# pyg-team/pyg-lib

Measured on AMD Instinct MI355X. Metric: segment_matmul GFLOP/s + sampled-edges/sec, 1/2/4/8 MI355X vs CPU ref, higher is better.
Workload: dtype bf16; 1 GPU; segment_matmul ogbn-mag-shaped: 154 relations, 21,111,007 rows, F_in=F_out=128 (BASELINE.json configs[1]); relations=154, rows=21111007, rows_per_gpu=21111007, F=128

## Files before the change

include/pyg_hip.h:

```cpp
#ifndef PYG_HIP_H_
#define PYG_HIP_H_

#include <stddef.h>
#include <stdint.h>

#ifdef __cplusplus
extern "C" {
#endif

#define PYG_HIP_API __attribute__((visibility("default")))

typedef enum {
  PYG_HIP_OK = 0,
  PYG_HIP_ERR_INVALID = -1,
  PYG_HIP_ERR_UNSUPPORTED = -2,
  PYG_HIP_ERR_RUNTIME = -3,
  PYG_HIP_ERR_WORKSPACE = -4
} pyg_hip_status;

typedef enum {
  PYG_F32 = 0,
  PYG_F64 = 1,
  PYG_F16 = 2,
  PYG_BF16 = 3,
  PYG_I8 = 4,
  PYG_U8 = 5,
  PYG_I16 = 6,
  PYG_I32 = 7,
  PYG_I64 = 8
} pyg_dtype;


#define PYG_HIP_ABI_VERSION 20
PYG_HIP_API int pyg_hip_abi_version(void);
PYG_HIP_API int64_t pyg_hip_version(void);
PYG_HIP_API const char* pyg_hip_last_error(void);
PYG_HIP_API const char* pyg_hip_arch(void);

PYG_HIP_API int pyg_hip_set_float_atomic_mode(int mode);
PYG_HIP_API const char* pyg_hip_last_accumulate_info(void);
PYG_HIP_API int pyg_hip_atomic_selftest(void* scratch, size_t scratch_bytes, int rounds, char* report, size_t report_cap,
                                        void* stream);


#define PYG_HIP_MM_SCHED_AUTO 0
#define PYG_HIP_MM_SCHED_CONTIGUOUS 1
#define PYG_HIP_MM_SCHED_CYCLIC 2
#define PYG_HIP_MM_SCHED_TICKET 3
#define PYG_HIP_MM_SCHED_GENERAL 4
#define PYG_HIP_MM_SCHED_NAIVE 5
#define PYG_HIP_MM_SCHED_RING 6
#define PYG_HIP_MM_SCHED_MASK 0xf
#define PYG_HIP_MM_F32_SPLIT 0x100

PYG_HIP_API size_t pyg_hip_matmul_workspace_size(int64_t num_groups);

// ... 45 lines not shown
} pyg_hip_rgcn_relation;

PYG_HIP_API size_t pyg_hip_rgcn_fused_workspace_size(int64_t num_relations, int64_t num_edges);

#define PYG_HIP_RGCN_CHECKED 1
#define PYG_HIP_RGCN_CAS 2
#define PYG_HIP_RGCN_DEFERRED 4
PYG_HIP_API int pyg_hip_rgcn_pending_error(void);
#define PYG_HIP_RGCN_GROUPED 8
PYG_HIP_API size_t pyg_hip_rgcn_grouped_workspace_size(const pyg_hip_rgcn_relation* relations, int64_t num_relations,
                                                       int64_t num_out_rows);
PYG_HIP_API int pyg_hip_rgcn_fused(int dtype, const void* x, int64_t num_x_rows, const pyg_hip_rgcn_relation* relations,
                                   int64_t num_relations, void* out, int64_t num_out_rows, int64_t K, int64_t M,
                                   int checked, void* workspace, size_t workspace_bytes, void* stream);
#define PYG_HIP_RGCN_ROUTE_UNSUPPORTED 0
#define PYG_HIP_RGCN_ROUTE_ATOMIC 1
#define PYG_HIP_RGCN_ROUTE_GROUPED_128 2
#define PYG_HIP_RGCN_ROUTE_GROUPED_SHAPE 3
#define PYG_HIP_RGCN_ROUTE_GROUPED_SMALL 4
#define PYG_HIP_RGCN_ROUTE_GROUPED_F32 5
#define PYG_HIP_RGCN_ROUTE_GROUPED_F32_SMALL 6
PYG_HIP_API int pyg_hip_rgcn_route(int dtype, int64_t K, int64_t M, int64_t num_relations, int flags);
PYG_HIP_API const char* pyg_hip_rgcn_last_route(void);


typedef struct {
  uint32_t state[624];
  int32_t left;
  uint32_t next;
} pyg_hip_mt19937;

typedef struct {
  void* user;
  void* (*alloc)(void* user, size_t bytes);
  void (*free)(void* user, void* ptr);
  void (*rng_blocks)(void* user, int64_t* words_host, int64_t num_blocks, int first);
  pyg_hip_mt19937* mt19937;
} pyg_hip_sampler_host;

typedef struct {
  const int64_t* rowptr;
  int64_t num_rows;
  const int64_t* col;
  int64_t num_cols;
  int32_t src_type;
  int32_t dst_type;
// ... 291 lines not shown
#define PYG_HIP_GRACLUS_TILE_SINGLE_THREADS 2
#define PYG_HIP_GRACLUS_TILE_SINGLE_MAX_NODES 3
#define PYG_HIP_GRACLUS_TILE_MULTI_THREADS 4
#define PYG_HIP_GRACLUS_TILE_BATCH 5
#define PYG_HIP_GRACLUS_TILE_SINGLE_MAX_EDGES 6
PYG_HIP_API int pyg_hip_graclus_route(int64_t N, int64_t E, int flags);
PYG_HIP_API const char* pyg_hip_graclus_last_route(void);
PYG_HIP_API int pyg_hip_graclus_tile(int which);
PYG_HIP_API size_t pyg_hip_graclus_workspace_size(int64_t N, int64_t E, int flags);
PYG_HIP_API int pyg_hip_graclus(const int64_t* rowptr, const int64_t* col, int weight_dtype, const void* weight, const int64_t* perm,
                                int64_t N, int64_t E, int flags, void* workspace, size_t workspace_bytes, int64_t* out, void* stream);
PYG_HIP_API int pyg_hip_graclus_pending_error(void);


PYG_HIP_API int pyg_hip_segment_csr(int op, int dtype, const void* src, const int64_t* indptr,
                                    int64_t indptr_slice_stride, void* out, int64_t* arg_out, int fresh,
                                    int64_t leading, int64_t rows, int64_t E, int64_t K, void* stream);

PYG_HIP_API size_t pyg_hip_csr_hub_workspace_size(int op, int dtype, int64_t leading, int64_t E, int64_t K);
PYG_HIP_API int pyg_hip_segment_csr_ws(int op, int dtype, const void* src, const int64_t* indptr,
                                       int64_t indptr_slice_stride, void* out, int64_t* arg_out, int fresh,
                                       int64_t leading, int64_t rows, int64_t E, int64_t K, void* workspace,
                                       size_t workspace_bytes, void* stream);

PYG_HIP_API int pyg_hip_gather_csr(int dtype, const void* src, const int64_t* indptr,
                                   int64_t indptr_slice_stride, void* out, int64_t leading, int64_t rows,
                                   int64_t E, int64_t K, void* stream);
PYG_HIP_API int pyg_hip_gather_csr_ws(int dtype, const void* src, const int64_t* indptr,
                                      int64_t indptr_slice_stride, void* out, int64_t leading, int64_t rows,
                                      int64_t E, int64_t K, void* workspace, size_t workspace_bytes, void* stream);

PYG_HIP_API int pyg_hip_softmax_csr(int dtype, const void* src, const int64_t* ptr, void* out, int64_t outer,
                                    int64_t D, int64_t inner, int64_t groups, void* stream);
PYG_HIP_API int pyg_hip_softmax_csr_backward(int dtype, const void* out, const void* out_grad,
                                             const int64_t* ptr, void* in_grad, int64_t outer, int64_t D,
                                             int64_t inner, int64_t groups, void* stream);

PYG_HIP_API const char* pyg_hip_csr_route(int family, int dtype, int64_t leading, int64_t rows, int64_t E, int64_t K,
                                          int flags, size_t workspace_bytes, unsigned misalign, int num_cus);
PYG_HIP_API const char* pyg_hip_csr_last_route(void);

PYG_HIP_API int64_t pyg_hip_hash_map_slots(int64_t n, double load_factor);
PYG_HIP_API int pyg_hip_hash_map_build(int key_dtype, const void* keys, int64_t n, uint64_t* table_keys,
                                       int64_t* table_vals, int64_t slots, int64_t* distinct_dev, void* stream);
PYG_HIP_API int pyg_hip_hash_map_get(int key_dtype, const void* query, int64_t m, const uint64_t* table_keys,
                                     const int64_t* table_vals, int64_t slots, int64_t* out, void* stream);
// ... 14 lines not shown
```

pyg_lib_amd/_capi.py:

```python
import ctypes
import os.path as osp

import torch

_HERE = osp.dirname(osp.abspath(__file__))
_LIB = None

OK = 0
ABI_VERSION = 20
DTYPES = {
    torch.float32: 0,
    torch.float64: 1,
    torch.float16: 2,
    torch.bfloat16: 3,
    torch.int8: 4,
    torch.uint8: 5,
    torch.int16: 6,
    torch.int32: 7,
    torch.int64: 8,
}


class Group(ctypes.Structure):
    _fields_ = [('input', ctypes.c_void_p), ('other', ctypes.c_void_p), ('out', ctypes.c_void_p),
                ('rows', ctypes.c_int64), ('k', ctypes.c_int32), ('m', ctypes.c_int32),
                ('other_trans', ctypes.c_int32), ('reserved', ctypes.c_int32)]


def lib_path() -> str:
    return osp.join(_HERE, 'libpyg_hip.so')


# ... 180 lines not shown
```

pyg_lib_amd/csrc/hip/csr.hip:

```cpp
#include "common.h"
#include "elem.h"
#include "csr_rows.h"

#include <algorithm>
#include <cstdint>
#include <type_traits>

namespace pyg_hip {
namespace {

enum { CSR_SUM = 0, CSR_MEAN = 1, CSR_MIN = 2, CSR_MAX = 3 };

template <typename T, int OP>
__device__ __forceinline__ typename Math<T>::acc_t minmax_identity() {
  return Math<T>::up(OP == CSR_MIN ? type_max<T>() : type_lowest<T>());
}

struct CsrShape {
  int64_t leading, rows, E, K;
  int64_t indptr_stride;
  int64_t long_cut = INT64_MAX;
  void* hub_ws = nullptr;
  size_t hub_ws_bytes = 0;
};
// ... 1176 lines not shown
}

size_t pyg_hip_csr_hub_workspace_size(int op, int dtype, int64_t leading, int64_t E, int64_t K) {
  CsrCall c{op, {}, leading, 0, E, K, false, 0, 0, 0, 0};
  if (leading < 0 || E < 0 || K <= 0 || op < 0 || op > CSR_GATHER || csr_type_of(dtype, &c.t) != PYG_HIP_OK) return 0;
  return csr_plan(c).ws_need;
}

int pyg_hip_segment_csr_ws(int op, int dtype, const void* src, const int64_t* indptr, int64_t indptr_slice_stride,
                           void* out, int64_t* arg_out, int fresh, int64_t leading, int64_t rows, int64_t E, int64_t K,
                           void* workspace, size_t workspace_bytes, void* stream_) {
  hipStream_t stream = static_cast<hipStream_t>(stream_);
  PYG_HIP_REQUIRE(leading >= 0 && rows >= 0 && E >= 0 && K >= 0, "segment_csr: negative size");
  if (csr_empty(CSR_SUM, leading, rows, E, K)) return note_empty();
  PYG_HIP_REQUIRE(op >= CSR_SUM && op <= CSR_MAX, "segment_csr: unknown reduction %d", op);
  PYG_HIP_REQUIRE(indptr && out && (src || E == 0), "segment_csr: NULL tensor");
  PYG_HIP_REQUIRE((op != CSR_MIN && op != CSR_MAX) || arg_out, "segment_csr: min/max need arg_out");
  PYG_HIP_REQUIRE(indptr_slice_stride == 0 || indptr_slice_stride >= rows + 1, "segment_csr: bad indptr stride");
  CsrShape s{leading, rows, E, K, indptr_slice_stride};
  s.hub_ws = workspace, s.hub_ws_bytes = workspace ? workspace_bytes : 0;
  PYG_DISPATCH_ALL(dtype, (run_segment<scalar_t>(op, src, indptr, nullptr, out, arg_out, fresh, s, stream)));
}

int pyg_hip_segment_csr(int op, int dtype, const void* src, const int64_t* indptr, int64_t indptr_slice_stride,
                        void* out, int64_t* arg_out, int fresh, int64_t leading, int64_t rows, int64_t E, int64_t K,
                        void* stream_) {
  return pyg_hip_segment_csr_ws(op, dtype, src, indptr, indptr_slice_stride, out, arg_out, fresh, leading, rows, E, K, nullptr, 0,
                                stream_);
}

int pyg_hip_gather_csr_ws(int dtype, const void* src, const int64_t* indptr, int64_t indptr_slice_stride, void* out,
                          int64_t leading, int64_t rows, int64_t E, int64_t K, void* workspace, size_t workspace_bytes,
                          void* stream_) {
  hipStream_t stream = static_cast<hipStream_t>(stream_);
  PYG_HIP_REQUIRE(leading >= 0 && rows >= 0 && E >= 0 && K >= 0, "gather_csr: negative size");
  if (csr_empty(CSR_GATHER, leading, rows, E, K)) return note_empty();
  PYG_HIP_REQUIRE(src && indptr && out, "gather_csr: NULL tensor");
  CsrShape s{leading, rows, E, K, indptr_slice_stride};
  s.hub_ws = workspace, s.hub_ws_bytes = workspace ? workspace_bytes : 0;
  PYG_DISPATCH_ALL(dtype, (run_gather_csr<scalar_t>(src, indptr, out, s, stream)));
}

int pyg_hip_gather_csr(int dtype, const void* src, const int64_t* indptr, int64_t indptr_slice_stride, void* out,
                       int64_t leading, int64_t rows, int64_t E, int64_t K, void* stream_) {
  return pyg_hip_gather_csr_ws(dtype, src, indptr, indptr_slice_stride, out, leading, rows, E, K, nullptr, 0, stream_);
}
// ... 25 lines not shown
```

pyg_lib_amd/rgcn.py:

```python
import os
import weakref
from typing import Dict, List, Optional, Tuple

import torch
from torch import Tensor
from torch.autograd.function import once_differentiable

from . import _capi, ops

EdgeType = Tuple[str, str, str]


def pending_index_error() -> int:
    return int(_capi.lib().pyg_hip_rgcn_pending_error())


_last_path = ['none']


def last_layer_path() -> str:
    return _last_path[0]


def last_layer_route() -> str:
# ... 66 lines not shown
    for et in edge_types:
        g, g_t, s, s_t = edge_roles(et, row_dict, col_dict, csc)
        counts.append(counts[-1] + g.numel())
        gather_idx.append(g + offsets[g_t] if offsets[g_t] else g)
        if num_out_rows is not None and s.numel() and not (x.is_cuda and torch.cuda.is_current_stream_capturing()):
            if int(s.max()) >= int(num_out_rows.get(s_t, 0)):
                raise RuntimeError(f"rgcn_layer: a scatter index of {et} is not below num_out_rows['{s_t}']")
        scatter_idx.append(s + ooff[s_t] if ooff[s_t] else s)
    total = ooff['__total__']
    if counts[-1] == 0:
        return x.new_zeros(total, weight.size(-1))
    gidx = torch.cat(gather_idx)
    sidx = torch.cat(scatter_idx)
    ptr = torch.tensor(counts, dtype=torch.long)
    feats = _GatherRows.apply(x, gidx)
    msgs = ops.segment_matmul(feats, ptr, weight)
    return ops.scatter_sum(msgs, sidx, dim=0, dim_size=total)


_DX_MODE = [os.environ.get('PYG_RGCN_DX', 'auto')]


def set_dx_mode(mode: str) -> str:
    if mode not in ('auto', 'grouped', 'atomic'):
        raise ValueError("dX mode must be 'auto', 'grouped' or 'atomic'")
    before, _DX_MODE[0] = _DX_MODE[0], mode
    return before


def _dx_grouped() -> bool:
    m = _DX_MODE[0]
    return m == 'grouped' or (m != 'atomic' and torch.are_deterministic_algorithms_enabled())


_ROUTE_ATOMIC, _FLAG_GROUPED = 1, 8


def _route(x: Tensor, weight: Tensor, relations: int, grouped: bool) -> int:
    code = _capi.DTYPES.get(x.dtype)
    if x.dim() != 2 or weight.dim() != 3 or code is None:
        return 0
    return _capi.lib().pyg_hip_rgcn_route(code, x.size(1), weight.size(2), relations, _FLAG_GROUPED if grouped else 0)


def _resolve_grouped(grouped: Optional[bool], scatter: List[Tensor]) -> bool:
    if grouped is None:
        from . import sampler
        grouped = all(sampler.rows_are_grouped(s) for s in scatter)
    return bool(grouped)


def _fusable(x: Tensor, weight: Tensor, grouped: bool = False, relations: int = 0) -> bool:
    if x.dim() != 2 or weight.dim() != 3:
        return False
    return (x.is_cuda and weight.size(1) == x.size(1) and weight.dtype == x.dtype and weight.device == x.device and
# ... 25 lines not shown


_transposed: Dict[Tuple, Tuple] = {}


def _transposed_sample(gather: List[Tensor], scatter: List[Tensor], gather_rows: int):
    key = tuple((id(t), t._version) for t in gather) + tuple((id(t), t._version) for t in scatter)
    hit = _transposed.get(key)
    if hit is not None and all(r() is t for r, t in zip(hit[0], list(gather) + list(scatter))):
        return hit[1], hit[2]
    counts = [g.numel() for g in gather]
    R = len(gather)
    keys = torch.cat([g + r * gather_rows if r else g for r, g in enumerate(gather)])
    skeys, perm = ops.index_sort(keys, max_value=max(R * gather_rows, 1))
    g_sorted = list(torch.split(skeys % gather_rows if R > 1 else skeys, counts))
    s_perm = list(torch.split(torch.cat(scatter)[perm], counts))
    if len(_transposed) >= 8:
        _transposed.pop(next(iter(_transposed)))
    refs = [weakref.ref(t) for t in list(gather) + list(scatter)]
    _transposed[key] = (refs, g_sorted, s_perm)
    return g_sorted, s_perm


def _dx_scatter(grad_out: Tensor, weight: Tensor, gather: List[Tensor], scatter: List[Tensor], goff: List[int],
                soff: List[int], rows: int, grows: Optional[List[int]] = None) -> Tensor:
    wt = weight.transpose(1, 2).contiguous()
    E = sum(g.numel() for g in gather)
    if E == 0:
        return grad_out.new_zeros(rows, weight.size(1))
    if _dx_grouped() and _fusable(grad_out, wt, True, len(gather)):
        g_sorted, s_perm = _transposed_sample(gather, scatter, rows)
        gx = grad_out.new_empty(rows, weight.size(1))
        torch.ops.pyg.rgcn_fused(grad_out, s_perm, g_sorted, soff, goff, wt, gx, True, grows)
        return gx
    if torch.are_deterministic_algorithms_enabled() or _route(grad_out, wt, len(gather), False) != _ROUTE_ATOMIC:
        ptr, gidx, sidx = _rel_ptr_and_indices(gather, scatter, goff, soff)
        msgs = ops.segment_matmul(ops.gather_coo(grad_out, sidx), ptr, wt)
        return ops.scatter_sum(msgs, gidx, dim=0, dim_size=rows)
    gx = grad_out.new_zeros(rows, weight.size(1))
    torch.ops.pyg.rgcn_fused(grad_out, scatter, gather, soff, goff, wt, gx)
    return gx


class _RGCNFused(torch.autograd.Function):

    @staticmethod
    def forward(ctx, x, weight, total, goff, soff, grouped, srows, grows, *index):
        R = len(index) // 2
        gather, scatter = list(index[:R]), list(index[R:])
        out = _fresh_out(x, total, weight.size(-1), grouped)
        torch.ops.pyg.rgcn_fused(x, gather, scatter, goff, soff, weight, out, grouped, srows)
        ctx.save_for_backward(x, weight, *index)
        ctx.meta = (goff, soff, R, grows)
        return out

    @staticmethod
    @once_differentiable
    def backward(ctx, grad_out):
        x, weight = ctx.saved_tensors[:2]
        index = ctx.saved_tensors[2:]
        goff, soff, R, grows = ctx.meta
        gather, scatter = list(index[:R]), list(index[R:])
        grad_out = grad_out.contiguous()
        gx = gw = None
        if ctx.needs_input_grad[0]:
            gx = _dx_scatter(grad_out, weight, gather, scatter, goff, soff, x.size(0), grows)
        if ctx.needs_input_grad[1]:
            ptr, gidx, sidx = _rel_ptr_and_indices(gather, scatter, goff, soff)
            if gidx.numel() == 0:
                gw = torch.zeros_like(weight)
            else:
                gw = torch.ops.pyg.segment_matmul_grad_other(ops.gather_coo(x, gidx), ptr, ops.gather_coo(grad_out, sidx))
        return (gx, gw, None, None, None, None, None, None) + (None,) * len(index)


class _RGCNFusedTables(torch.autograd.Function):

    @staticmethod
    def forward(ctx, weight, T, gtype, soff, grouped, out_rows, srows, *tensors):
        feat, node_id = list(tensors[:T]), list(tensors[T:2 * T])
        index = tensors[2 * T:]
        R = len(index) // 2
        gather, scatter = list(index[:R]), list(index[R:])
        n_t = [t.numel() for t in node_id]
        out = _fresh_out(feat[0], out_rows, weight.size(-1), grouped)
        torch.ops.pyg.rgcn_fused_tables(feat, node_id, gtype, gather, scatter, soff, weight, out, grouped, srows)
        ctx.save_for_backward(weight, *tensors)
        ctx.meta = (T, gtype, soff, R, n_t)
        return out

    @staticmethod
    @once_differentiable
    def backward(ctx, grad_out):
        weight = ctx.saved_tensors[0]
        tensors = ctx.saved_tensors[1:]
        T, gtype, soff, R, n_t = ctx.meta
        feat, node_id = list(tensors[:T]), list(tensors[T:2 * T])
        index = tensors[2 * T:]
        gather, scatter = list(index[:R]), list(index[R:])
        grad_out = grad_out.contiguous()
        toff = [0]
        for n in n_t:
            toff.append(toff[-1] + n)
        goff = [toff[t] for t in gtype]
        gw = None
        gfeat = [None] * T
        if ctx.needs_input_grad[0]:
            ptr, gidx, sidx = _rel_ptr_and_indices(gather, scatter, goff, soff)
            if gidx.numel() == 0:
                gw = torch.zeros_like(weight)
            else:
                xb = torch.cat([f[n] for f, n in zip(feat, node_id)])
                gw = torch.ops.pyg.segment_matmul_grad_other(ops.gather_coo(xb, gidx), ptr, ops.gather_coo(grad_out, sidx))
        if any(ctx.needs_input_grad[7 + t] for t in range(T)):
            gx = _dx_scatter(grad_out, weight, gather, scatter, goff, soff, toff[-1], [max(n_t[t], 1) for t in gtype])
            for t in range(T):
                if ctx.needs_input_grad[7 + t]:
                    gfeat[t] = torch.zeros_like(feat[t]).index_add_(0, node_id[t], gx[toff[t]:toff[t + 1]])
        return (gw, None, None, None, None, None, None) + tuple(gfeat) + (None,) * (len(tensors) - T)


def rgcn_layer_fused(x: Tensor, offsets: Dict[str, int], row_dict: Dict[EdgeType, Tensor],
                     col_dict: Dict[EdgeType, Tensor], edge_types: List[EdgeType], weight: Tensor,
                     csc: bool = False, grouped: Optional[bool] = None,
                     num_out_rows: Optional[Dict[str, int]] = None) -> Tensor:
    ooff = out_offsets(offsets, num_out_rows)
    total = ooff['__total__']
    roles = [edge_roles(et, row_dict, col_dict, csc) for et in edge_types]
    grouped = _resolve_grouped(grouped, [r[2] for r in roles]) and _fusable(x, weight, True, len(roles))
    if not (grouped or _fusable(x, weight, False, len(roles))) or (torch.are_deterministic_algorithms_enabled() and not grouped):
        return rgcn_layer(x, offsets, row_dict, col_dict, edge_types, weight, csc, num_out_rows)
    gather, scatter = [r[0] for r in roles], [r[2] for r in roles]
    goff, soff = [offsets[r[1]] for r in roles], [ooff[r[3]] for r in roles]
    srows = _scatter_rows(ooff, roles, edge_types)
    _last_path[0] = 'grouped' if grouped else 'atomic'
    if torch.is_grad_enabled() and (x.requires_grad or weight.requires_grad):
        trows = _type_rows(offsets)
        grows = [max(trows[r[1]], 1) for r in roles]
# ... 34 lines not shown
```

Baseline: 397,200 GFLOP/s.

## Compute RGCN backward dW and dX over scatter-row runs instead of per-edge

Adds a run-decomposition kernel that groups consecutive edges sharing a scatter row (capped at 32 per run). dW pre-sums gathered x rows per run and multiplies by one grad_out row per run, and dX multiplies grad_out once per run and then does a CSR index-sum over source rows. The intent is to cut per-edge GEMM rows and gathers in the backward pass, at the cost of new indexing kernels and cached run metadata keyed on tensor identity. It only touches the RGCN fused backward, not the segment_matmul forward throughput being measured.

```diff
diff --git a/include/pyg_hip.h b/include/pyg_hip.h
--- a/include/pyg_hip.h
+++ b/include/pyg_hip.h
@@ -31,7 +31,7 @@
 } pyg_dtype;
 
 
-#define PYG_HIP_ABI_VERSION 20
+#define PYG_HIP_ABI_VERSION 21
 PYG_HIP_API int pyg_hip_abi_version(void);
 PYG_HIP_API int64_t pyg_hip_version(void);
 PYG_HIP_API const char* pyg_hip_last_error(void);
@@ -123,6 +123,14 @@
 #define PYG_HIP_RGCN_ROUTE_GROUPED_F32_SMALL 6
 PYG_HIP_API int pyg_hip_rgcn_route(int dtype, int64_t K, int64_t M, int64_t num_relations, int flags);
 PYG_HIP_API const char* pyg_hip_rgcn_last_route(void);
+
+PYG_HIP_API size_t pyg_hip_rgcn_runs_workspace_size(int64_t num_edges);
+PYG_HIP_API int pyg_hip_rgcn_runs(const pyg_hip_rgcn_relation* relations, int64_t num_relations, int64_t max_len,
+                                  int64_t* run_ptr, int64_t* run_row, int64_t* rel_run_ptr, int32_t* run_of_edge,
+                                  int64_t* gather_rows, void* workspace, size_t workspace_bytes, void* stream);
+PYG_HIP_API int pyg_hip_rgcn_run_rows(int dtype, const void* x, int64_t num_x_rows, int64_t K, const int64_t* gather_rows,
+                                      const int64_t* run_ptr, const int64_t* run_row, int64_t num_runs, const void* grad_out,
+                                      int64_t num_out_rows, int64_t M, float* agg, float* grow, void* stream);
 
 
 typedef struct {
@@ -460,6 +468,9 @@
                                        int64_t indptr_slice_stride, void* out, int64_t* arg_out, int fresh,
                                        int64_t leading, int64_t rows, int64_t E, int64_t K, void* workspace,
                                        size_t workspace_bytes, void* stream);
+PYG_HIP_API int pyg_hip_segment_csr_index_sum(int dtype, const void* src, const int64_t* index, const int64_t* indptr, void* out,
+                                              int64_t rows, int64_t E, int64_t K, void* workspace, size_t workspace_bytes,
+                                              void* stream);
 
 PYG_HIP_API int pyg_hip_gather_csr(int dtype, const void* src, const int64_t* indptr,
                                    int64_t indptr_slice_stride, void* out, int64_t leading, int64_t rows,
diff --git a/pyg_lib_amd/_capi.py b/pyg_lib_amd/_capi.py
--- a/pyg_lib_amd/_capi.py
+++ b/pyg_lib_amd/_capi.py
@@ -7,7 +7,7 @@
 _LIB = None
 
 OK = 0
-ABI_VERSION = 20
+ABI_VERSION = 21
 DTYPES = {
     torch.float32: 0,
     torch.float64: 1,
diff --git a/pyg_lib_amd/csrc/binding/pyg_binding_rgcn_runs.cpp b/pyg_lib_amd/csrc/binding/pyg_binding_rgcn_runs.cpp
--- /dev/null
+++ b/pyg_lib_amd/csrc/binding/pyg_binding_rgcn_runs.cpp
@@ -0,0 +1,223 @@
+#include <ATen/ATen.h>
+#include <torch/library.h>
+
+#include <tuple>
+#include <vector>
+
+#include "binding_common.h"
+
+namespace pyg_amd {
+namespace {
+
+using Runs = std::tuple<Tensor, Tensor, Tensor, Tensor, Tensor>;
+
+int64_t check_runs(const at::TensorList scatter_index, at::IntArrayRef scatter_offset, const at::TensorList gather_index,
+                   at::IntArrayRef gather_offset, int64_t max_len) {
+  const size_t R = scatter_index.size();
+  TORCH_CHECK(R > 0 && gather_index.size() == R && scatter_offset.size() == R && gather_offset.size() == R,
+              "rgcn_runs: one scatter / gather index vector and offset per relation expected (at least one relation)");
+  TORCH_CHECK(max_len >= 1, "rgcn_runs: max_len must be positive");
+  int64_t E = 0;
+  for (size_t r = 0; r < R; ++r) {
+    for (const Tensor* t : {&scatter_index[r], &gather_index[r]})
+      TORCH_CHECK(t->dim() == 1 && t->scalar_type() == at::kLong && t->device() == scatter_index[0].device(),
+                  "rgcn_runs: index vectors must be 1-D int64 tensors on one device");
+    TORCH_CHECK(scatter_index[r].numel() == gather_index[r].numel(), "rgcn_runs: index vectors of a relation differ in length");
+    E += scatter_index[r].numel();
+  }
+  return E;
+}
+
+void check_dw_runs(const Tensor& x, const Tensor& gather_rows, const Tensor& grad_out, const Tensor& run_ptr, const Tensor& run_row,
+                   const Tensor& rel_run_ptr, int64_t num_runs) {
+  TORCH_CHECK(x.dim() == 2 && grad_out.dim() == 2 && x.scalar_type() == grad_out.scalar_type() && x.device() == grad_out.device(),
+              "rgcn_dw_runs: expected x [N, K] and grad_out [N_out, M] of one type on one device");
+  TORCH_CHECK(x.scalar_type() == at::kBFloat16 || x.scalar_type() == at::kHalf || x.scalar_type() == at::kFloat,
+              "rgcn_dw_runs: float32 / bfloat16 / float16 only (got ", x.scalar_type(), ")");
+  for (const Tensor* t : {&gather_rows, &run_ptr, &run_row, &rel_run_ptr})
+    TORCH_CHECK(t->dim() == 1 && t->scalar_type() == at::kLong && t->device() == x.device() && t->is_contiguous(),
+                "rgcn_dw_runs: gather_rows, run_ptr, run_row and rel_run_ptr must be contiguous int64 vectors on the device of x");
+  TORCH_CHECK(num_runs >= 0 && num_runs <= gather_rows.numel() && run_ptr.numel() > num_runs && run_row.numel() >= num_runs &&
+                  rel_run_ptr.numel() >= 1,
+              "rgcn_dw_runs: expected gather_rows [E >= P], run_ptr [> P], run_row [>= P], rel_run_ptr [R + 1]");
+  TORCH_CHECK(x.size(0) > 0 && grad_out.size(0) > 0 || num_runs == 0, "rgcn_dw_runs: runs over tensors without rows");
+}
+
+void check_dx_runs(const Tensor& grad_out, const Tensor& weight, const Tensor& run_row, const Tensor& rel_run_ptr, int64_t num_runs,
+                   const Tensor& src_index, const Tensor& indptr, int64_t rows) {
+  TORCH_CHECK(grad_out.dim() == 2 && weight.dim() == 3 && weight.size(2) == grad_out.size(1) &&
+                  weight.scalar_type() == grad_out.scalar_type() && weight.device() == grad_out.device(),
+              "rgcn_dx_runs: expected grad_out [N_out, M] and weight [R, K, M] of one type on one device");
+  TORCH_CHECK(grad_out.scalar_type() == at::kBFloat16 || grad_out.scalar_type() == at::kHalf || grad_out.scalar_type() == at::kFloat,
+              "rgcn_dx_runs: float32 / bfloat16 / float16 only (got ", grad_out.scalar_type(), ")");
+  for (const Tensor* t : {&run_row, &rel_run_ptr, &src_index, &indptr})
+    TORCH_CHECK(t->dim() == 1 && t->scalar_type() == at::kLong && t->device() == grad_out.device() && t->is_contiguous(),
+                "rgcn_dx_runs: run_row, rel_run_ptr, src_index and indptr must be contiguous int64 vectors on the device of grad_out");
+  TORCH_CHECK(num_runs >= 0 && run_row.numel() >= num_runs && rel_run_ptr.numel() == weight.size(0) + 1 && rows >= 0 &&
+                  indptr.numel() == rows + 1 && (num_runs == 0 || grad_out.size(0) > 0),
+              "rgcn_dx_runs: expected run_row [>= P], rel_run_ptr [R + 1], indptr [rows + 1]");
+}
+
+Runs rgcn_runs_kernel(const at::TensorList scatter_index, at::IntArrayRef scatter_offset, const at::TensorList gather_index,
+                      at::IntArrayRef gather_offset, int64_t max_len) {
+  PYG_TRACE("pyg::rgcn_runs");
+  const int64_t E = check_runs(scatter_index, scatter_offset, gather_index, gather_offset, max_len);
+  const size_t R = scatter_index.size();
+  const Tensor& like = scatter_index[0];
+  DeviceGuard guard(like.device());
+  std::vector<pyg_hip_rgcn_relation> rels(R);
+  std::vector<Tensor> keep;
+  for (size_t r = 0; r < R; ++r) {
+    keep.push_back(scatter_index[r].contiguous());
+    keep.push_back(gather_index[r].contiguous());
+    rels[r] = pyg_hip_rgcn_relation{};
+    rels[r].scatter_index = keep[2 * r].data_ptr<int64_t>();
+    rels[r].gather_index = keep[2 * r + 1].data_ptr<int64_t>();
+    rels[r].num_edges = keep[2 * r].numel();
+    rels[r].scatter_offset = scatter_offset[r];
+    rels[r].gather_offset = gather_offset[r];
+  }
+  const auto longs = like.options().dtype(at::kLong);
+  Tensor run_ptr = at::empty({E + 1}, longs), run_row = at::empty({E}, longs), rel_run_ptr = at::empty({(int64_t)R + 1}, longs);
+  Tensor run_of_edge = at::empty({E}, longs.dtype(at::kInt)), gather_rows = at::empty({E}, longs);
+  Tensor ws = at::empty({(int64_t)pyg_hip_rgcn_runs_workspace_size(E)}, longs.dtype(at::kByte));
+  check_status(pyg_hip_rgcn_runs(rels.data(), (int64_t)R, max_len, run_ptr.data_ptr<int64_t>(), run_row.data_ptr<int64_t>(),
+                                 rel_run_ptr.data_ptr<int64_t>(), run_of_edge.data_ptr<int32_t>(), gather_rows.data_ptr<int64_t>(),
+                                 ws.data_ptr(), (size_t)ws.numel(), current_stream(like)));
+  return {run_ptr, run_row, rel_run_ptr, run_of_edge, gather_rows};
+}
+
+Tensor rgcn_dw_runs_kernel(const Tensor& x, const Tensor& gather_rows, const Tensor& grad_out, const Tensor& run_ptr,
+                           const Tensor& run_row, const Tensor& rel_run_ptr, int64_t num_runs) {
+  PYG_TRACE("pyg::rgcn_dw_runs");
+  check_dw_runs(x, gather_rows, grad_out, run_ptr, run_row, rel_run_ptr, num_runs);
+  const int64_t R = rel_run_ptr.numel() - 1, K = x.size(1), M = grad_out.size(1), P = num_runs;
+  if (R == 0 || P == 0) return at::zeros({R, K, M}, x.options());
+  DeviceGuard guard(x.device());
+  const Tensor xc = x.contiguous(), gc = grad_out.contiguous();
+  const auto floats = x.options().dtype(at::kFloat);
+  Tensor agg = at::empty({P, K}, floats), grow = at::empty({P, M}, floats), dw = at::empty({R, K, M}, floats);
+  check_status(pyg_hip_rgcn_run_rows(dtype_code(x.scalar_type()), xc.data_ptr(), xc.size(0), K, gather_rows.data_ptr<int64_t>(),
+                                     run_ptr.data_ptr<int64_t>(), run_row.data_ptr<int64_t>(), P, gc.data_ptr(), gc.size(0), M,
+                                     agg.data_ptr<float>(), grow.data_ptr<float>(), current_stream(x)));
+  Tensor ws = at::empty({(int64_t)pyg_hip_segment_matmul_dw_workspace_size(R, K, M)}, floats.dtype(at::kByte));
+  check_status(pyg_hip_segment_matmul_dw(PYG_F32, agg.data_ptr(), rel_run_ptr.data_ptr<int64_t>(), 1, grow.data_ptr(), dw.data_ptr(),
+                                         P, K, M, R, ws.data_ptr(), (size_t)ws.numel(), current_stream(x)));
+  return dw.to(x.scalar_type());
+}
+
+Tensor rgcn_dx_runs_kernel(const Tensor& grad_out, const Tensor& weight, const Tensor& run_row, const Tensor& rel_run_ptr,
+                           int64_t num_runs, const Tensor& src_index, const Tensor& indptr, int64_t rows) {
+  PYG_TRACE("pyg::rgcn_dx_runs");
+  check_dx_runs(grad_out, weight, run_row, rel_run_ptr, num_runs, src_index, indptr, rows);
+  const int64_t R = weight.size(0), K = weight.size(1), M = weight.size(2), P = num_runs, E = src_index.numel();
+  if (rows == 0 || K == 0 || P == 0 || E == 0) return at::zeros({rows, K}, grad_out.options());
+  DeviceGuard guard(grad_out.device());
+  const int dt = dtype_code(grad_out.scalar_type());
+  const Tensor gc = grad_out.contiguous(), wt = weight.transpose(1, 2).contiguous();
+  Tensor gst = at::empty({P, M}, gc.options()), T = at::empty({P, K}, gc.options()), dx = at::empty({rows, K}, gc.options());
+  check_status(pyg_hip_gather_coo(dt, gc.data_ptr(), run_row.data_ptr<int64_t>(), gst.data_ptr(), 1, P, M, gc.size(0), current_stream(gc)));
+  const auto bytes = gc.options().dtype(at::kByte);
+  Tensor ws = at::empty({(int64_t)pyg_hip_matmul_workspace_size(R)}, bytes);
+  check_status(pyg_hip_segment_matmul(dt, gst.data_ptr(), rel_run_ptr.data_ptr<int64_t>(), 1, wt.data_ptr(), nullptr, T.data_ptr(), P, M, K, R,
+                                      ws.data_ptr(), (size_t)ws.numel(), 0, current_stream(gc)));
+  Tensor hub = at::empty({(int64_t)pyg_hip_csr_hub_workspace_size(0, dt, 1, E, K)}, bytes);
+  check_status(pyg_hip_segment_csr_index_sum(dt, T.data_ptr(), src_index.data_ptr<int64_t>(), indptr.data_ptr<int64_t>(), dx.data_ptr(),
+                                             rows, E, K, hub.numel() ? hub.data_ptr() : nullptr, (size_t)hub.numel(), current_stream(gc)));
+  return dx;
+}
+
+Tensor rgcn_dx_runs_cpu(const Tensor& grad_out, const Tensor& weight, const Tensor& run_row, const Tensor& rel_run_ptr,
+                        int64_t num_runs, const Tensor& src_index, const Tensor& indptr, int64_t rows) {
+  check_dx_runs(grad_out, weight, run_row, rel_run_ptr, num_runs, src_index, indptr, rows);
+  const int64_t R = weight.size(0), K = weight.size(1), P = num_runs;
+  if (rows == 0 || K == 0 || P == 0 || src_index.numel() == 0) return at::zeros({rows, K}, grad_out.options());
+  const Tensor gst = grad_out.index_select(0, run_row.narrow(0, 0, P)).to(at::kFloat);
+  const int64_t* rel = rel_run_ptr.data_ptr<int64_t>();
+  std::vector<Tensor> parts;
+  for (int64_t r = 0; r < R; ++r)
+    parts.push_back(at::matmul(gst.narrow(0, rel[r], rel[r + 1] - rel[r]), weight[r].to(at::kFloat).t()));
+  const Tensor T = at::cat(parts).to(grad_out.scalar_type()).to(at::kFloat);
+  const Tensor row_of = at::repeat_interleave(at::arange(rows, indptr.options()), indptr.narrow(0, 1, rows) - indptr.narrow(0, 0, rows));
+  return at::zeros({rows, K}, gst.options()).index_add_(0, row_of, T.index_select(0, src_index)).to(grad_out.scalar_type());
+}
+
+Runs rgcn_runs_cpu(const at::TensorList scatter_index, at::IntArrayRef scatter_offset, const at::TensorList gather_index,
+                   at::IntArrayRef gather_offset, int64_t max_len) {
+  const int64_t E = check_runs(scatter_index, scatter_offset, gather_index, gather_offset, max_len);
+  const size_t R = scatter_index.size();
+  const auto longs = scatter_index[0].options().dtype(at::kLong);
+  Tensor run_ptr = at::zeros({E + 1}, longs), run_row = at::zeros({E}, longs), rel_run_ptr = at::zeros({(int64_t)R + 1}, longs);
+  Tensor run_of_edge = at::zeros({E}, longs.dtype(at::kInt)), gather_rows = at::zeros({E}, longs);
+  int64_t* rp = run_ptr.data_ptr<int64_t>();
+  int64_t* rr = run_row.data_ptr<int64_t>();
+  int64_t* rel = rel_run_ptr.data_ptr<int64_t>();
+  int32_t* roe = run_of_edge.data_ptr<int32_t>();
+  int64_t* gr = gather_rows.data_ptr<int64_t>();
+  int64_t P = 0, pos = 0;
+  for (size_t r = 0; r < R; ++r) {
+    const Tensor s = scatter_index[r].contiguous(), g = gather_index[r].contiguous();
+    const int64_t* sp = s.data_ptr<int64_t>();
+    const int64_t* gp = g.data_ptr<int64_t>();
+    rel[r] = P;
+    int64_t first = 0;
+    for (int64_t j = 0; j < s.numel(); ++j, ++pos) {
+      if (j == 0 || sp[j] != sp[j - 1]) first = j;
+      if ((j - first) % max_len == 0) {
+        rp[P] = pos;
+        rr[P] = sp[j] + scatter_offset[r];
+        ++P;
+      }
+      roe[pos] = (int32_t)(P - 1);
+      gr[pos] = gp[j] + gather_offset[r];
+    }
+  }
+  rel[R] = P;
+  rp[P] = E;
+  return {run_ptr, run_row, rel_run_ptr, run_of_edge, gather_rows};
+}
+
+Tensor rgcn_dw_runs_cpu(const Tensor& x, const Tensor& gather_rows, const Tensor& grad_out, const Tensor& run_ptr,
+                        const Tensor& run_row, const Tensor& rel_run_ptr, int64_t num_runs) {
+  check_dw_runs(x, gather_rows, grad_out, run_ptr, run_row, rel_run_ptr, num_runs);
+  const int64_t R = rel_run_ptr.numel() - 1, K = x.size(1), M = grad_out.size(1), P = num_runs;
+  if (R == 0 || P == 0) return at::zeros({R, K, M}, x.options());
+  const Tensor ptr = run_ptr.narrow(0, 0, P + 1);
+  const Tensor run_id = at::repeat_interleave(at::arange(P, ptr.options()), ptr.narrow(0, 1, P) - ptr.narrow(0, 0, P));
+  const Tensor rows = x.to(at::kFloat).index_select(0, gather_rows.narrow(0, 0, run_id.numel()));
+  const Tensor agg = at::zeros({P, K}, x.options().dtype(at::kFloat)).index_add_(0, run_id, rows);
+  const Tensor grow = grad_out.to(at::kFloat).index_select(0, run_row.narrow(0, 0, P));
+  const int64_t* rel = rel_run_ptr.data_ptr<int64_t>();
+  std::vector<Tensor> parts;
+  for (int64_t r = 0; r < R; ++r)
+    parts.push_back(at::matmul(agg.narrow(0, rel[r], rel[r + 1] - rel[r]).t(), grow.narrow(0, rel[r], rel[r + 1] - rel[r])));
+  return at::stack(parts).to(x.scalar_type());
+}
+
+}
+
+TORCH_LIBRARY_FRAGMENT(pyg, m) {
+  m.def(TORCH_SELECTIVE_SCHEMA(
+      "pyg::rgcn_runs(Tensor[] scatter_index, int[] scatter_offset, Tensor[] gather_index, int[] gather_offset, int max_len) -> "
+      "(Tensor, Tensor, Tensor, Tensor, Tensor)"));
+  m.def(TORCH_SELECTIVE_SCHEMA(
+      "pyg::rgcn_dw_runs(Tensor x, Tensor gather_rows, Tensor grad_out, Tensor run_ptr, Tensor run_row, Tensor rel_run_ptr, "
+      "int num_runs) -> Tensor"));
+  m.def(TORCH_SELECTIVE_SCHEMA(
+      "pyg::rgcn_dx_runs(Tensor grad_out, Tensor weight, Tensor run_row, Tensor rel_run_ptr, int num_runs, Tensor src_index, "
+      "Tensor indptr, int rows) -> Tensor"));
+}
+
+TORCH_LIBRARY_IMPL(pyg, CUDA, m) {
+  m.impl(TORCH_SELECTIVE_NAME("pyg::rgcn_runs"), TORCH_FN(rgcn_runs_kernel));
+  m.impl(TORCH_SELECTIVE_NAME("pyg::rgcn_dw_runs"), TORCH_FN(rgcn_dw_runs_kernel));
+  m.impl(TORCH_SELECTIVE_NAME("pyg::rgcn_dx_runs"), TORCH_FN(rgcn_dx_runs_kernel));
+}
+
+TORCH_LIBRARY_IMPL(pyg, CPU, m) {
+  m.impl(TORCH_SELECTIVE_NAME("pyg::rgcn_runs"), TORCH_FN(rgcn_runs_cpu));
+  m.impl(TORCH_SELECTIVE_NAME("pyg::rgcn_dw_runs"), TORCH_FN(rgcn_dw_runs_cpu));
+  m.impl(TORCH_SELECTIVE_NAME("pyg::rgcn_dx_runs"), TORCH_FN(rgcn_dx_runs_cpu));
+}
+
+}
diff --git a/pyg_lib_amd/csrc/hip/csr.hip b/pyg_lib_amd/csrc/hip/csr.hip
--- a/pyg_lib_amd/csrc/hip/csr.hip
+++ b/pyg_lib_amd/csrc/hip/csr.hip
@@ -1222,6 +1222,15 @@
   PYG_DISPATCH_ALL(dtype, (run_segment<scalar_t>(op, src, indptr, nullptr, out, arg_out, fresh, s, stream)));
 }
 
+int pyg_hip_segment_csr_index_sum(int dtype, const void* src, const int64_t* index, const int64_t* indptr, void* out,
+                                  int64_t rows, int64_t E, int64_t K, void* workspace, size_t workspace_bytes, void* stream_) {
+  hipStream_t stream = static_cast<hipStream_t>(stream_);
+  PYG_HIP_REQUIRE(rows >= 0 && E >= 0 && K >= 0, "segment_csr_index_sum: negative size");
+  if (csr_empty(CSR_SUM, 1, rows, E, K)) return note_empty();
+  PYG_HIP_REQUIRE(indptr && out && ((src && index) || E == 0), "segment_csr_index_sum: NULL tensor");
+  return segment_csr_sum(dtype, src, indptr, 0, index, out, 1, rows, E, K, 1, stream, workspace, workspace ? workspace_bytes : 0);
+}
+
 int pyg_hip_segment_csr(int op, int dtype, const void* src, const int64_t* indptr, int64_t indptr_slice_stride,
                         void* out, int64_t* arg_out, int fresh, int64_t leading, int64_t rows, int64_t E, int64_t K,
                         void* stream_) {
diff --git a/pyg_lib_amd/csrc/hip/rgcn_runs.hip b/pyg_lib_amd/csrc/hip/rgcn_runs.hip
--- /dev/null
+++ b/pyg_lib_amd/csrc/hip/rgcn_runs.hip
@@ -0,0 +1,253 @@
+#include "csr_rows.h"
+#include "scan.h"
+
+namespace pyg_hip {
+namespace {
+
+constexpr int kRunsMaxRel = 32;
+constexpr int kRunsRowBits = 40;
+constexpr int64_t kRunsRowMask = (1LL << kRunsRowBits) - 1;
+
+struct RunsRel {
+  const int64_t* scatter[kRunsMaxRel];
+  const int64_t* gather[kRunsMaxRel];
+  int64_t soff[kRunsMaxRel], goff[kRunsMaxRel];
+  int64_t start[kRunsMaxRel + 1];
+};
+
+__global__ __launch_bounds__(256) void runs_keys_kernel(RunsRel t, int64_t E, int64_t* __restrict__ keys,
+                                                        int64_t* __restrict__ gather_rows) {
+  const int64_t i = (int64_t)blockIdx.x * 256 + threadIdx.x;
+  if (i >= E) return;
+  const int64_t* s = t.scatter[0];
+  const int64_t* g = t.gather[0];
+  int64_t so = t.soff[0], go = t.goff[0], st = t.start[0], rel = 0;
+#pragma unroll
+  for (int r = 1; r < kRunsMaxRel; ++r) {
+    const bool in = i >= t.start[r];
+    s = in ? t.scatter[r] : s;
+    g = in ? t.gather[r] : g;
+    so = in ? t.soff[r] : so;
+    go = in ? t.goff[r] : go;
+    st = in ? t.start[r] : st;
+    rel = in ? r : rel;
+  }
+  keys[i] = (rel << kRunsRowBits) | ((s[i - st] + so) & kRunsRowMask);
+  if (gather_rows) gather_rows[i] = g[i - st] + go;
+}
+
+struct MaxOp {
+  __host__ __device__ int64_t operator()(int64_t a, int64_t b) const { return a > b ? a : b; }
+  __host__ __device__ static int64_t identity() { return -1; }
+};
+
+struct StretchLoad {
+  const int64_t* keys;
+  __device__ int64_t operator()(int64_t i) const { return (i == 0 || keys[i] != keys[i - 1]) ? i : -1; }
+};
+struct StretchStore {
+  int64_t* first;
+  __device__ void operator()(int64_t i, int64_t before, int64_t v) const { first[i] = v > before ? v : before; }
+};
+
+struct RunLoad {
+  const int64_t* first;
+  int64_t max_len;
+  __device__ int64_t operator()(int64_t i) const { return (i - first[i]) % max_len == 0 ? 1 : 0; }
+};
+struct RunStore {
+  const int64_t* keys;
+  int64_t* run_ptr;
+  int64_t* run_row;
+  int64_t* rel_run_ptr;
+  int32_t* run_of_edge;
+  __device__ void operator()(int64_t i, int64_t before, int64_t v) const {
+    run_of_edge[i] = (int32_t)(before + v - 1);
+    if (v == 0) return;
+    const int64_t key = keys[i];
+    run_ptr[before] = i;
+    run_row[before] = key & kRunsRowMask;
+    const int64_t rel = key >> kRunsRowBits, prev = i == 0 ? -1 : keys[i - 1] >> kRunsRowBits;
+    for (int64_t r = prev + 1; r <= rel; ++r) rel_run_ptr[r] = before;
+  }
+};
+
+__global__ void runs_close_kernel(const int64_t* __restrict__ keys, int R, int64_t E, const int64_t* __restrict__ total,
+                                  int64_t* __restrict__ run_ptr, int64_t* __restrict__ rel_run_ptr) {
+  const int64_t P = *total;
+  const int r = threadIdx.x;
+  const int64_t last = E > 0 ? keys[E - 1] >> kRunsRowBits : -1;
+  if (r == 0) run_ptr[P] = E;
+  if (r <= R && r > last) rel_run_ptr[r] = P;
+}
+
+struct RunsWs {
+  size_t keys, first, tiles, total, bytes;
+};
+RunsWs carve_runs(int64_t E) {
+  const size_t n = (size_t)(E > 0 ? E : 1);
+  RunsWs w;
+  w.keys = 0;
+  w.first = align_up(sizeof(int64_t) * n, 256);
+  w.tiles = w.first + align_up(sizeof(int64_t) * n, 256);
+  w.total = w.tiles + align_up(sizeof(int64_t) * ((n + kScanTile - 1) / kScanTile), 256);
+  w.bytes = w.total + 256;
+  return w;
+}
+
+template <typename T, int LPR>
+__global__ __launch_bounds__(256) void run_rows_kernel(const T* __restrict__ x, int64_t x_rows, int64_t K,
+                                                       const int64_t* __restrict__ gather_rows, const int64_t* __restrict__ run_ptr,
+                                                       const int64_t* __restrict__ run_row, int64_t P_runs,
+                                                       const T* __restrict__ gout, int64_t out_rows, int64_t M,
+                                                       float* __restrict__ agg, float* __restrict__ grow) {
+  constexpr int V = 16 / (int)sizeof(T);
+  constexpr int U = 8;
+  using P = Pack<T, V>;
+  const int64_t p = ((int64_t)blockIdx.x * 256 + threadIdx.x) / LPR;
+  if (p >= P_runs) return;
+  const int64_t col = (int64_t)(threadIdx.x & (LPR - 1)) * V;
+  const int64_t a = run_ptr[p], b = run_ptr[p + 1];
+  if (grow != nullptr && col < M) {
+    int64_t row = run_row[p];
+    row = row < 0 ? 0 : (row >= out_rows ? out_rows - 1 : row);
+    const P g = *reinterpret_cast<const P*>(gout + row * M + col);
+    float* o = grow + p * M + col;
+#pragma unroll
+    for (int i = 0; i < V; i += 4)
+      *reinterpret_cast<float4*>(o + i) = make_float4(Math<T>::up(g.v[i]), Math<T>::up(g.v[i + 1]), Math<T>::up(g.v[i + 2]),
+                                                      Math<T>::up(g.v[i + 3]));
+  }
+  if (col >= K) return;
+  float acc[V];
+#pragma unroll
+  for (int i = 0; i < V; ++i) acc[i] = sum_identity<float>();
+  for (int64_t e0 = a; e0 < b; e0 += U) {
+    int64_t pp[U];
+    P xx[U];
+#pragma unroll
+    for (int u = 0; u < U; ++u) pp[u] = gather_rows[e0 + u < b ? e0 + u : e0];
+    pin_all(pp);
+#pragma unroll
+    for (int u = 0; u < U; ++u) {
+      const int64_t row = pp[u] < 0 ? 0 : (pp[u] >= x_rows ? x_rows - 1 : pp[u]);
+      xx[u] = *reinterpret_cast<const P*>(x + row * K + col);
+    }
+    pin_all(xx);
+#pragma unroll
+    for (int u = 0; u < U; ++u) {
+      if (e0 + u >= b) break;
+#pragma unroll
+      for (int i = 0; i < V; ++i) acc[i] += Math<T>::up(xx[u].v[i]);
+    }
+  }
+  float* o = agg + p * K + col;
+#pragma unroll
+  for (int i = 0; i < V; i += 4) *reinterpret_cast<float4*>(o + i) = make_float4(acc[i], acc[i + 1], acc[i + 2], acc[i + 3]);
+}
+
+template <typename T>
+int run_rows_launch(const void* x, int64_t x_rows, int64_t K, const int64_t* gather_rows, const int64_t* run_ptr,
+                    const int64_t* run_row, int64_t P, const void* gout, int64_t out_rows, int64_t M, float* agg, float* grow,
+                    hipStream_t stream) {
+  constexpr int V = 16 / (int)sizeof(T);
+  const int64_t chunks = (K > M ? K : M) / V;
+  const int lpr = chunks <= 4 ? 4 : chunks <= 8 ? 8 : chunks <= 16 ? 16 : 32;
+  const dim3 grid((unsigned)((P * lpr + 255) / 256)), block(256);
+  const T* xp = static_cast<const T*>(x);
+  const T* gp = static_cast<const T*>(gout);
+#define PYG_RUN_ROWS(LPR) \
+  hipLaunchKernelGGL((run_rows_kernel<T, LPR>), grid, block, 0, stream, xp, x_rows, K, gather_rows, run_ptr, run_row, P, gp, out_rows, M, agg, grow)
+  if (lpr == 4) PYG_RUN_ROWS(4);
+  else if (lpr == 8) PYG_RUN_ROWS(8);
+  else if (lpr == 16) PYG_RUN_ROWS(16);
+  else PYG_RUN_ROWS(32);
+#undef PYG_RUN_ROWS
+  PYG_HIP_CHECK(hipGetLastError());
+  return PYG_HIP_OK;
+}
+
+}
+}
+
+using namespace pyg_hip;
+
+extern "C" {
+
+size_t pyg_hip_rgcn_runs_workspace_size(int64_t num_edges) { return carve_runs(num_edges).bytes; }
+
+int pyg_hip_rgcn_runs(const pyg_hip_rgcn_relation* rels, int64_t R, int64_t max_len, int64_t* run_ptr, int64_t* run_row,
+                      int64_t* rel_run_ptr, int32_t* run_of_edge, int64_t* gather_rows, void* workspace, size_t workspace_bytes,
+                      void* stream_) {
+  hipStream_t stream = static_cast<hipStream_t>(stream_);
+  if (R < 0 || R > kRunsMaxRel) return fail(PYG_HIP_ERR_UNSUPPORTED, "rgcn_runs: 0 ... %d relations (got %lld)", kRunsMaxRel, (long long)R);
+  PYG_HIP_REQUIRE(R == 0 || rels != nullptr, "rgcn_runs: null relations");
+  PYG_HIP_REQUIRE(max_len >= 1, "rgcn_runs: max_len must be positive");
+  PYG_HIP_REQUIRE(run_ptr && rel_run_ptr, "rgcn_runs: null output");
+  RunsRel t;
+  int64_t E = 0;
+  for (int r = 0; r < kRunsMaxRel; ++r) {
+    t.start[r] = E;
+    t.scatter[r] = t.gather[r] = nullptr;
+    t.soff[r] = t.goff[r] = 0;
+    if (r >= R) continue;
+    PYG_HIP_REQUIRE(rels[r].num_edges >= 0, "rgcn_runs: negative edge count");
+    PYG_HIP_REQUIRE(rels[r].num_edges == 0 || (rels[r].scatter_index && (rels[r].gather_index || !gather_rows)),
+                    "rgcn_runs: null index vector");
+    t.scatter[r] = rels[r].scatter_index;
+    t.gather[r] = rels[r].gather_index;
+    t.soff[r] = rels[r].scatter_offset;
+    t.goff[r] = rels[r].gather_offset;
+    E += rels[r].num_edges;
+    if (E >= (1LL << 31)) return fail(PYG_HIP_ERR_UNSUPPORTED, "rgcn_runs: 2^31 or more edges");
+  }
+  t.start[kRunsMaxRel] = E;
+  PYG_HIP_REQUIRE(E == 0 || (run_row && run_of_edge), "rgcn_runs: null output");
+  const RunsWs lay = carve_runs(E);
+  if (workspace == nullptr || workspace_bytes < lay.bytes)
+    return fail(PYG_HIP_ERR_WORKSPACE, "rgcn_runs: workspace of %zu bytes needed, got %zu", lay.bytes, workspace_bytes);
+  char* ws = static_cast<char*>(workspace);
+  int64_t* keys = reinterpret_cast<int64_t*>(ws + lay.keys);
+  int64_t* first = reinterpret_cast<int64_t*>(ws + lay.first);
+  int64_t* tiles = reinterpret_cast<int64_t*>(ws + lay.tiles);
+  int64_t* total = reinterpret_cast<int64_t*>(ws + lay.total);
+  int rc = PYG_HIP_OK;
+  if (E > 0) {
+    hipLaunchKernelGGL(runs_keys_kernel, dim3((unsigned)((E + 255) / 256)), dim3(256), 0, stream, t, E, keys, gather_rows);
+    rc = device_scan<int64_t, MaxOp>(StretchLoad{keys}, StretchStore{first}, E, tiles, total, stream);
+    if (rc != PYG_HIP_OK) return rc;
+  }
+  rc = device_scan<int64_t, SumOp>(RunLoad{first, max_len}, RunStore{keys, run_ptr, run_row, rel_run_ptr, run_of_edge}, E, tiles, total,
+                                   stream);
+  if (rc != PYG_HIP_OK) return rc;
+  hipLaunchKernelGGL(runs_close_kernel, dim3(1), dim3(64), 0, stream, (const int64_t*)keys, (int)R, E, (const int64_t*)total, run_ptr,
+                     rel_run_ptr);
+  PYG_HIP_CHECK(hipGetLastError());
+  return PYG_HIP_OK;
+}
+
+int pyg_hip_rgcn_run_rows(int dtype, const void* x, int64_t num_x_rows, int64_t K, const int64_t* gather_rows, const int64_t* run_ptr,
+                          const int64_t* run_row, int64_t P, const void* grad_out, int64_t num_out_rows, int64_t M, float* agg,
+                          float* grow, void* stream_) {
+  hipStream_t stream = static_cast<hipStream_t>(stream_);
+  const bool half = dtype == PYG_BF16 || dtype == PYG_F16;
+  if (!half && dtype != PYG_F32) return fail(PYG_HIP_ERR_UNSUPPORTED, "rgcn_run_rows: bf16 / f16 / f32 only");
+  const int64_t V = half ? 8 : 4, top = half ? 256 : 128;
+  if (K < V || K > top || K % V != 0 || M < V || M > top || M % V != 0)
+    return fail(PYG_HIP_ERR_UNSUPPORTED, "rgcn_run_rows: K = %lld, M = %lld are not multiples of %lld up to %lld", (long long)K,
+                (long long)M, (long long)V, (long long)top);
+  PYG_HIP_REQUIRE(P >= 0, "rgcn_run_rows: negative run count");
+  if (P == 0) return PYG_HIP_OK;
+  PYG_HIP_REQUIRE(P < (1LL << 31) / 32, "rgcn_run_rows: too many runs");
+  PYG_HIP_REQUIRE(x && gather_rows && run_ptr && agg && num_x_rows > 0, "rgcn_run_rows: null tensor");
+  PYG_HIP_REQUIRE(grow == nullptr || (grad_out && run_row && num_out_rows > 0), "rgcn_run_rows: null tensor");
+  PYG_HIP_REQUIRE(((reinterpret_cast<uintptr_t>(x) | reinterpret_cast<uintptr_t>(grad_out) | reinterpret_cast<uintptr_t>(agg) |
+                    reinterpret_cast<uintptr_t>(grow)) & 15) == 0, "rgcn_run_rows: misaligned tensor");
+  if (dtype == PYG_BF16)
+    return run_rows_launch<bf16_t>(x, num_x_rows, K, gather_rows, run_ptr, run_row, P, grad_out, num_out_rows, M, agg, grow, stream);
+  if (dtype == PYG_F16)
+    return run_rows_launch<f16_t>(x, num_x_rows, K, gather_rows, run_ptr, run_row, P, grad_out, num_out_rows, M, agg, grow, stream);
+  return run_rows_launch<float>(x, num_x_rows, K, gather_rows, run_ptr, run_row, P, grad_out, num_out_rows, M, agg, grow, stream);
+}
+
+}
diff --git a/pyg_lib_amd/rgcn.py b/pyg_lib_amd/rgcn.py
--- a/pyg_lib_amd/rgcn.py
+++ b/pyg_lib_amd/rgcn.py
@@ -112,15 +112,15 @@
 
 
 def set_dx_mode(mode: str) -> str:
-    if mode not in ('auto', 'grouped', 'atomic'):
-        raise ValueError("dX mode must be 'auto', 'grouped' or 'atomic'")
+    if mode not in ('auto', 'grouped', 'atomic', 'rows'):
+        raise ValueError("dX mode must be 'auto', 'grouped', 'atomic' or 'rows'")
     before, _DX_MODE[0] = _DX_MODE[0], mode
     return before
 
 
 def _dx_grouped() -> bool:
     m = _DX_MODE[0]
-    return m == 'grouped' or (m != 'atomic' and torch.are_deterministic_algorithms_enabled())
+    return m in ('grouped', 'rows') or (m != 'atomic' and torch.are_deterministic_algorithms_enabled())
 
 
 _ROUTE_ATOMIC, _FLAG_GROUPED = 1, 8
@@ -192,12 +192,72 @@
     return g_sorted, s_perm
 
 
+_RUN_LEN = 32
+_RUN_MAX_RELATIONS = 32
+_DW_MODE = [os.environ.get('PYG_RGCN_DW', 'runs')]
+_runs: Dict[Tuple, Tuple] = {}
+
+
+def set_dw_mode(mode: str) -> str:
+    if mode not in ('runs', 'edges'):
+        raise ValueError("dW mode must be 'runs' or 'edges'")
+    before, _DW_MODE[0] = _DW_MODE[0], mode
+    return before
+
+
+def _sample_runs(gather: List[Tensor], scatter: List[Tensor], goff: List[int], soff: List[int]):
+    key = tuple((id(t), t._version) for t in gather) + tuple((id(t), t._version) for t in scatter) + tuple(goff) + tuple(soff)
+    hit = _runs.get(key)
+    if hit is not None and all(r() is t for r, t in zip(hit[0], list(gather) + list(scatter))):
+        return hit[1]
+    out = torch.ops.pyg.rgcn_runs(list(scatter), list(soff), list(gather), list(goff), _RUN_LEN)
+    val = tuple(out) + (int(out[2][-1]),)
+    if len(_runs) >= 8:
+        _runs.pop(next(iter(_runs)))
+    _runs[key] = ([weakref.ref(t) for t in list(gather) + list(scatter)], val)
+    return val
+
+
+def _weight_grad(x: Tensor, grad_out: Tensor, weight: Tensor, gather: List[Tensor], scatter: List[Tensor], goff: List[int],
+                 soff: List[int], grouped: bool) -> Tensor:
+    if sum(g.numel() for g in gather) == 0:
+        return torch.zeros_like(weight)
+    if (grouped and _DW_MODE[0] != 'edges' and len(gather) <= _RUN_MAX_RELATIONS and x.is_cuda and
+            not torch.cuda.is_current_stream_capturing()):
+        run_ptr, run_row, rel_run_ptr, _, gather_rows, P = _sample_runs(gather, scatter, goff, soff)
+        return torch.ops.pyg.rgcn_dw_runs(x, gather_rows, grad_out, run_ptr, run_row, rel_run_ptr, P)
+    ptr, gidx, sidx = _rel_ptr_and_indices(gather, scatter, goff, soff)
+    return torch.ops.pyg.segment_matmul_grad_other(ops.gather_coo(x, gidx), ptr, ops.gather_coo(grad_out, sidx))
+
+
+_by_source: Dict[Tuple, Tuple] = {}
+
+
+def _edges_by_source(gather: List[Tensor], scatter: List[Tensor], goff: List[int], soff: List[int], rows: int):
+    key = tuple((id(t), t._version) for t in gather) + tuple((id(t), t._version) for t in scatter) + tuple(goff) + tuple(soff) + (rows,)
+    hit = _by_source.get(key)
+    if hit is not None and all(r() is t for r, t in zip(hit[0], list(gather) + list(scatter))):
+        return hit[1]
+    _, _, _, run_of_edge, gather_rows, _ = _sample_runs(gather, scatter, goff, soff)
+    skeys, perm = ops.index_sort(gather_rows, max_value=max(rows, 1))
+    val = (run_of_edge[perm].long(), torch._convert_indices_from_coo_to_csr(skeys, rows))
+    if len(_by_source) >= 8:
+        _by_source.pop(next(iter(_by_source)))
+    _by_source[key] = ([weakref.ref(t) for t in list(gather) + list(scatter)], val)
+    return val
+
+
 def _dx_scatter(grad_out: Tensor, weight: Tensor, gather: List[Tensor], scatter: List[Tensor], goff: List[int],
-                soff: List[int], rows: int, grows: Optional[List[int]] = None) -> Tensor:
-    wt = weight.transpose(1, 2).contiguous()
+                soff: List[int], rows: int, grows: Optional[List[int]] = None, runs: bool = False) -> Tensor:
     E = sum(g.numel() for g in gather)
     if E == 0:
         return grad_out.new_zeros(rows, weight.size(1))
+    if (_dx_grouped() and runs and _DX_MODE[0] != 'rows' and len(gather) <= _RUN_MAX_RELATIONS and grad_out.is_cuda and
+            not torch.cuda.is_current_stream_capturing()):
+        _, run_row, rel_run_ptr, _, _, P = _sample_runs(gather, scatter, goff, soff)
+        src_index, indptr = _edges_by_source(gather, scatter, goff, soff, rows)
+        return torch.ops.pyg.rgcn_dx_runs(grad_out, weight, run_row, rel_run_ptr, P, src_index, indptr, rows)
+    wt = weight.transpose(1, 2).contiguous()
     if _dx_grouped() and _fusable(grad_out, wt, True, len(gather)):
         g_sorted, s_perm = _transposed_sample(gather, scatter, rows)
         gx = grad_out.new_empty(rows, weight.size(1))
@@ -221,7 +281,7 @@
         out = _fresh_out(x, total, weight.size(-1), grouped)
         torch.ops.pyg.rgcn_fused(x, gather, scatter, goff, soff, weight, out, grouped, srows)
         ctx.save_for_backward(x, weight, *index)
-        ctx.meta = (goff, soff, R, grows)
+        ctx.meta = (goff, soff, R, grows, grouped)
         return out
 
     @staticmethod
@@ -229,18 +289,14 @@
     def backward(ctx, grad_out):
         x, weight = ctx.saved_tensors[:2]
         index = ctx.saved_tensors[2:]
-        goff, soff, R, grows = ctx.meta
+        goff, soff, R, grows, grouped = ctx.meta
         gather, scatter = list(index[:R]), list(index[R:])
         grad_out = grad_out.contiguous()
         gx = gw = None
         if ctx.needs_input_grad[0]:
-            gx = _dx_scatter(grad_out, weight, gather, scatter, goff, soff, x.size(0), grows)
+            gx = _dx_scatter(grad_out, weight, gather, scatter, goff, soff, x.size(0), grows, grouped)
         if ctx.needs_input_grad[1]:
-            ptr, gidx, sidx = _rel_ptr_and_indices(gather, scatter, goff, soff)
-            if gidx.numel() == 0:
-                gw = torch.zeros_like(weight)
-            else:
-                gw = torch.ops.pyg.segment_matmul_grad_other(ops.gather_coo(x, gidx), ptr, ops.gather_coo(grad_out, sidx))
+            gw = _weight_grad(x, grad_out, weight, gather, scatter, goff, soff, grouped)
         return (gx, gw, None, None, None, None, None, None) + (None,) * len(index)
 
 
@@ -256,7 +312,7 @@
         out = _fresh_out(feat[0], out_rows, weight.size(-1), grouped)
         torch.ops.pyg.rgcn_fused_tables(feat, node_id, gtype, gather, scatter, soff, weight, out, grouped, srows)
         ctx.save_for_backward(weight, *tensors)
-        ctx.meta = (T, gtype, soff, R, n_t)
+        ctx.meta = (T, gtype, soff, R, n_t, grouped)
         return out
 
     @staticmethod
@@ -264,7 +320,7 @@
     def backward(ctx, grad_out):
         weight = ctx.saved_tensors[0]
         tensors = ctx.saved_tensors[1:]
-        T, gtype, soff, R, n_t = ctx.meta
+        T, gtype, soff, R, n_t, grouped = ctx.meta
         feat, node_id = list(tensors[:T]), list(tensors[T:2 * T])
         index = tensors[2 * T:]
         gather, scatter = list(index[:R]), list(index[R:])
@@ -276,14 +332,10 @@
         gw = None
         gfeat = [None] * T
         if ctx.needs_input_grad[0]:
-            ptr, gidx, sidx = _rel_ptr_and_indices(gather, scatter, goff, soff)
-            if gidx.numel() == 0:
-                gw = torch.zeros_like(weight)
-            else:
-                xb = torch.cat([f[n] for f, n in zip(feat, node_id)])
-                gw = torch.ops.pyg.segment_matmul_grad_other(ops.gather_coo(xb, gidx), ptr, ops.gather_coo(grad_out, sidx))
+            xb = torch.cat([f[n] for f, n in zip(feat, node_id)])
+            gw = _weight_grad(xb, grad_out, weight, gather, scatter, goff, soff, grouped)
         if any(ctx.needs_input_grad[7 + t] for t in range(T)):
-            gx = _dx_scatter(grad_out, weight, gather, scatter, goff, soff, toff[-1], [max(n_t[t], 1) for t in gtype])
+            gx = _dx_scatter(grad_out, weight, gather, scatter, goff, soff, toff[-1], [max(n_t[t], 1) for t in gtype], grouped)
             for t in range(T):
                 if ctx.needs_input_grad[7 + t]:
                     gfeat[t] = torch.zeros_like(feat[t]).index_add_(0, node_id[t], gx[toff[t]:toff[t + 1]])
```

After: 391,500 GFLOP/s. 0.986x the previous value.
